# soedinglab/BaMMmotif2

Hardware: AMD Instinct MI355X
Metric: EM seq-positions/sec (and iterations/sec), 1Mx200bp k=2 W=20 (higher is better)
Workload: dtype f32

## Files before the change

### bammmotif2_amd/build.py

```python
from __future__ import annotations

import contextlib
import fcntl
import json
import os
import re
import shutil
import subprocess

HERE = os.path.dirname(os.path.abspath(__file__))
CSRC = os.path.join(HERE, "csrc")
LIB = os.path.join(HERE, "libbamm_em.so")
SOURCES = ["model.hip", "kernels.hip", "grouped.hip", "grouped_long.hip", "grouped_xl.hip", "grouped_mix.hip", "grouped_mix1.hip", "mask.hip", "seed.hip", "long_seq.hip", "prep.hip", "negs.hip", "occ.hip", "sites.hip", "fdr.hip", "ctx.cpp", "seqs.cpp", "plan.cpp", "em_pass.cpp", "em.cpp",
           "score.cpp", "occurrences.cpp", "sites.cpp", "fdr_stats.cpp", "comm.cpp", "pack.cpp"]
HEADERS = [os.path.join(CSRC, "common.h"), os.path.join(CSRC, "device_utils.h"), os.path.join(CSRC, "grouped_kernel.h"), os.path.join(CSRC, "mixed_kernel.h"), os.path.join(CSRC, "update_kernel.h"), os.path.join(CSRC, "phase_clock.h"),
           os.path.join(HERE, "..", "include", "bamm_em.h")]
FLAGS = ["--offload-arch=gfx950", "-O3", "-std=c++17", "-fPIC", "-ffp-contract=off", "-fno-slp-vectorize",
         "-Wall", "-Wno-unused-result", "-Rpass-analysis=kernel-resource-usage"]
_IEEE = ["-fhip-fp32-correctly-rounded-divide-sqrt", "-fno-gpu-flush-denormals-to-zero"]
TU_FLAGS = {"occ.hip": _IEEE, "fdr.hip": _IEEE, "grouped_long.hip": ["-falign-functions=16384"], "grouped_xl.hip": ["-falign-functions=16384"], "kernels.hip": ["-falign-functions=16384"]}
OBJDIR = os.path.join(HERE, "build")
RESOURCES = os.path.join(OBJDIR, "resources.json")


def _stem(src: str) -> str:
    stem, ext = os.path.splitext(src)
    return stem + "_host" if ext == ".cpp" and stem + ".hip" in SOURCES else stem


def _obj(src: str) -> str:
    return os.path.join(OBJDIR, _stem(src) + ".o")


def _remarks(src: str) -> str:
    return os.path.join(OBJDIR, _stem(src) + ".remarks")


def _diagnostics(text: str) -> str:
    keep, skip = [], 0
    for line in text.splitlines():
        if "[-Rpass-analysis=kernel-resource-usage]" in line:
            skip = 2 if "Function Name" in line else 0
            continue
        if skip:
            skip -= 1
            continue
        keep.append(line)
    return "\n".join(keep).strip()
# ... 166 lines not shown
```

### bammmotif2_amd/csrc/common.h

```cpp
#pragma once
#include <hip/hip_runtime.h>

#include <cstdint>
#include <cstdio>
#include <cstring>
#include <map>
#include <memory>
#include <string>
#include <vector>

#include "../../include/bamm_em.h"

namespace bamm {

void set_error(const char* fmt, ...);

#define BAMM_HIP(expr)                                                                        \
    do {                                                                                      \
        hipError_t e_ = (expr);                                                               \
        if (e_ != hipSuccess) {                                                               \
            ::bamm::set_error("%s failed: %s (%s:%d)", #expr, hipGetErrorString(e_), __FILE__, \
                              __LINE__);                                                      \
            return BAMM_ERR_HIP;                                                              \
        }                                                                                     \
// ... 122 lines not shown
    const float* v_old;
    float* s;
    float* q;
    float* q_out;
    float* status;
    float* trace;
    uint32_t trace_cap;
    uint32_t* iteration;
    int32_t optimize_q;
    double n_seqs_override;
    uint32_t* stop;
    float epsilon;
    float llh_prev;
    int32_t llh_prev_from_status;
    const float* llh_in;
    float* llh_out;
    uint32_t opt_iteration;
    unsigned long long* status_mirror;
    double*   partial;
    uint32_t* ticket;
};
constexpr uint32_t kUpdateMaxBlocks = 1024;

inline size_t update_lds_bytes(uint32_t K, uint32_t W) {
    auto even = [](size_t x) { return (x + 1) & ~size_t(1); };
    return (even(v_size(K, W)) + even((size_t)(K + 1) * W) + even(bg_size(K))) * sizeof(float) + (16 + 4) * sizeof(double);
}
inline bool update_fits_lds(uint32_t K, uint32_t W) { return ipow4(K + 1) * W <= 2048u && update_lds_bytes(K, W) <= 60u * 1024u; }

struct GrpKernelArgs {
    EmKernelArgs e;
    GrpGeom g;
    const uint4* xrec;
    unsigned long long* fix_log;
    uint32_t fix_log_cap;
    uint32_t fused;
    uint32_t upd_off;
    float*   s_block;
    UpdateArgs upd;
    PeerArgs peer;
};

bool grp_geometry(uint32_t K, uint32_t W, uint32_t G, int M, uint32_t waves, bool accum, uint32_t logC, uint32_t layout,
                  GrpGeom* out);
bool grp_plan(uint32_t K, uint32_t W, int M, uint32_t waves, bool many_exceptions, bool enough_work, uint32_t forced_G,
              int forced_layout, uint32_t* G, uint32_t* logC, uint32_t* layout);
bool grp_supported_class(int M, uint32_t K);
int launch_em_grp_long(int mclass, bool accum, bool write_r, const GrpKernelArgs& a, uint32_t blocks, uint32_t threads,
                       hipStream_t st);
int launch_em_grp_xl(int mclass, bool accum, bool write_r, const GrpKernelArgs& a, uint32_t blocks, uint32_t threads,
                     hipStream_t st);
uint32_t grp_max_threads(int M);
bool mix_geometry(uint32_t K, uint32_t W, int M, uint32_t waves, bool accum, GrpGeom* out);
int launch_em_mix(int mclass, bool accum, bool write_r, const GrpKernelArgs& a, uint32_t blocks, uint32_t threads, hipStream_t st);
int launch_em_mix1(int mclass, bool accum, bool write_r, const GrpKernelArgs& a, uint32_t blocks, uint32_t threads, hipStream_t st);
int launch_em_grp(int mclass, bool accum, bool write_r, const GrpKernelArgs& a, uint32_t blocks, uint32_t threads,
                  hipStream_t st);

struct SeedKernelArgs {
    SeqView  sv;
    uint32_t K, W, Y;
    uint32_t max_len, vsize;
    uint32_t table_bytes, count_bytes, wave_bytes;
    const float* score;
    float    q;
    const double* u;
    int*     counts;
    uint32_t* z_out;
    unsigned char* wave_scratch;
};
size_t seed_global_scratch_bytes(const SeedKernelArgs& a, uint32_t num_cus);
int launch_seed_pwm(SeedKernelArgs a, uint32_t num_cus, hipStream_t st);

struct ScoreKernelArgs {
    SeqView  sv;
    uint32_t K, W, Y;
    const float* s;
    float*   mops;
    const uint64_t* mops_off;
    float*   zoops;
    uint32_t* z;
};


struct OccCand {
    unsigned long long window;
    float    score;
    float    higher, lower;
    uint32_t fp;
};
// ... 134 lines not shown
```

### bammmotif2_amd/csrc/em.cpp

```cpp

#include <atomic>
#include <cmath>

#include "handles.h"

using namespace bamm;

int bamm::dense_r_on_device(bamm_em* em, uint64_t begin, uint64_t end, DevTemps& tmp, DenseR* out) {
    bamm_seqs* s = em->seqs;
    hipStream_t st = em->ctx->stream;
    const uint64_t base = s->h_pos_off[begin], total = s->h_pos_off[end] - base;
    if (em->mask_done) {
        *out = DenseR{em->d_mask_r, 0, false};
        return BAMM_OK;
    }
    if (em->sliced) {
        uint8_t* saved_mask = em->d_mask;
        em->d_mask = nullptr;
        const uint32_t used = em->events_used, pass_no = em->pass_no;
        int rc2 = run_accumulate(em, false, true, true);
        em->events_used = used; em->pass_no = pass_no;
        em->d_mask = saved_mask;
        if (rc2) return rc2;
        *out = DenseR{em->d_state, 0, !em->e_fused};
// ... 3 lines not shown
    int rc = tmp.scratch(&d_r, total);
    if (rc) return rc;
    if (hipMemsetAsync(d_r, 0, total * sizeof(float), st) != hipSuccess) { set_error("hipMemsetAsync failed"); return BAMM_ERR_HIP; }
    for (size_t b = 0; b < em->ebuckets.size() && !rc; b++) {
        const EmBucket& bk = em->ebuckets[b];
        EmKernelArgs a{};
        a.sv = make_view(s, em->exc, bk.d_idx, bk.count, nullptr);
        a.K = em->prm.K; a.W = em->prm.W; a.Y = em->Y;
        a.s = em->s_last; a.q = em->q_last;
        a.acc = nullptr;
        a.r_out = d_r; a.r_base = base; a.seq_begin = (uint32_t)begin; a.seq_end = (uint32_t)end;
        a.fix_scale = 1.0f;
        if (bk.mclass == kLongClass) { rc = launch_long_em(a, false, true, false, bk.blocks, st); continue; }
        rc = launch_fused(em, bk, false, true, a, bucket_threads(em->ctx, bk), st);
    }
    *out = DenseR{d_r, base, false};
    return rc;
}

extern "C" {

int bamm_em_destroy(bamm_em* em) {
    if (!em) return BAMM_OK;
    (void)hipSetDevice(em->ctx->device);
    (void)hipStreamSynchronize(em->ctx->stream);
    for (void* p : {(void*)em->d_vbg, (void*)em->d_A, (void*)em->d_v, (void*)em->d_n, (void*)em->d_s, (void*)em->d_qbuf[0],
                    (void*)em->d_status, (void*)em->d_trace, (void*)em->d_iteration, (void*)em->d_mask, (void*)em->d_acc_ring,
                    (void*)em->d_v_alt, (void*)em->d_llh[0], (void*)em->d_s_block, (void*)em->d_nnz, (void*)em->d_upd_partial, (void*)em->d_upd_ticket,
                    (void*)em->d_state, (void*)em->d_list_r, (void*)em->d_list_p, (void*)em->d_list_n, (void*)em->d_s_alt, (void*)em->d_fix_log,
                    (void*)em->d_qbuf[1], (void*)em->d_qbuf[2],
                    (void*)em->d_mask_r, (void*)em->d_mask_bits, (void*)em->d_mask_hist, (void*)em->d_mask_sel, (void*)em->d_mask_qseq,
                    (void*)em->d_mask_partial_n, (void*)em->d_mask_partial_stat})
        scratch_free(em->ctx, p);
    for (uint32_t* p : em->owned_idx) (void)hipFree(p);
    if (em->h_status) (void)hipHostFree(em->h_status);
    (void)hipFree(em->d_stop);
    (void)hipFree(em->d_peer_words);
    (void)hipFree(em->d_comm_words);
    for (hipEvent_t e : em->opt_events) if (e) (void)hipEventDestroy(e);
    for (auto& ev : em->events) { (void)hipEventDestroy(ev.first); (void)hipEventDestroy(ev.second); }
    bamm_seqs_destroy(em->seqs);
    delete em;
    return BAMM_OK;
}

int bamm_em_create(bamm_ctx* c, bamm_seqs* seqs, const bamm_em_params* prm, const float* vbg, const float* A,
                   const float* v_init, const uint8_t* seq_mask, bamm_em** out) {
    if (!c || !seqs || !prm || !vbg || !A || !v_init || !out) { set_error("bamm_em_create: null argument"); return BAMM_ERR_ARG; }
    *out = nullptr;
    if (seqs->ctx != c) { set_error("sequence set belongs to another context"); return BAMM_ERR_ARG; }
    if (prm->K > BAMM_MAX_ORDER) { set_error("order %u > %d (kmer_ spans 11 bases)", prm->K, BAMM_MAX_ORDER); return BAMM_ERR_ARG; }
    if (prm->W == 0) { set_error("motif width 0"); return BAMM_ERR_ARG; }
    if (seqs->n && seqs->min_len < prm->W) {
        set_error("a sequence of length %u is shorter than the motif (W=%u); the reference drops those before EM (mainBaMM.cpp:75-83)",
                  seqs->min_len, prm->W);
        return BAMM_ERR_ARG;
    }
    const uint32_t Y = (uint32_t)ipow4(prm->K + 1);
    BAMM_HIP(hipSetDevice(c->device));
    bamm_em* em = new bamm_em();
    em->ctx = c;
    em->seqs = seqs;
    { std::lock_guard<std::mutex> lock(seqs->mu); seqs->refs++; }
    em->prm = *prm;
    if (em->prm.max_iterations == 0) em->prm.max_iterations = 1000;
    em->Y = Y;
// ... 562 lines not shown
```

### bammmotif2_amd/csrc/em_pass.cpp

```cpp

#include <cmath>

#include "handles.h"

namespace bamm {

static int event_pair(bamm_em* em) {
    if (em->events_used == em->events.size()) {
        hipEvent_t a, b;
        BAMM_HIP(hipEventCreate(&a));
        BAMM_HIP(hipEventCreate(&b));
        em->events.emplace_back(a, b);
        em->event_passes.push_back(1u);
    }
    return BAMM_OK;
}
int record_event(bamm_em* em, bool start) {
    if (em->timing_every == BAMM_TIMING_WHOLE_CALL) {
        if (!start) return BAMM_OK;
        em->pass_no++;
        if (!em->region_open) {
            if (int rc = event_pair(em)) return rc;
            BAMM_HIP(hipEventRecord(em->events[em->events_used].first, em->ctx->stream));
            em->region_open = true;
// ... 9 lines not shown
    if (!em->timing_now) return BAMM_OK;
    if (start) {
        if (int rc = event_pair(em)) return rc;
        BAMM_HIP(hipEventRecord(em->events[em->events_used].first, em->ctx->stream));
    } else {
        BAMM_HIP(hipEventRecord(em->events[em->events_used].second, em->ctx->stream));
        em->event_passes[em->events_used] = 1u;
        em->events_used++;
    }
    return BAMM_OK;
}
int close_timed_region(bamm_em* em) {
    if (!em->region_open) return BAMM_OK;
    em->region_open = false;
    BAMM_HIP(hipEventRecord(em->events[em->events_used].second, em->ctx->stream));
    em->event_passes[em->events_used] = em->region_passes;
    em->events_used++;
    return BAMM_OK;
}

int launch_fused(bamm_em* em, const EmBucket& eb, bool accum, bool write_r, EmKernelArgs& a, uint32_t threads,
                 hipStream_t st, const UpdateArgs* fuse) {
    if (!eb.grouped) {
        a.logC = eb.logc;
        a.sparse_cap = accum ? eb.sparse_cap : 0u;
        a.sparse_wave_bytes = accum ? eb.sparse_bytes : 0u;
        return launch_em_seq(eb.mclass, accum, write_r, a, eb.blocks, threads, st);
    }
    GrpKernelArgs ga{};
    a.logC = eb.logc;
    a.sparse_cap = 0; a.sparse_wave_bytes = 0;
    ga.e = a;
    ga.xrec = eb.d_xrec;
    if (!grp_geometry(em->prm.K, em->prm.W, eb.G, kMClasses[eb.mclass], threads / 64u, accum, accum ? eb.logc : 0u, eb.layout, &ga.g)) {
        set_error("grouped kernel geometry does not fit (K=%u W=%u)", em->prm.K, em->prm.W);
        return BAMM_ERR_UNSUPPORTED;
    }
    if ((em->prm.K == 3u || (eb.layout & 8u)) && accum) {
        const size_t waves = (size_t)eb.blocks * (threads / 64u);
        const size_t cap = ((eb.count + waves - 1) / waves) * std::min<size_t>(64, (size_t)ga.g.Bv * ga.g.T);
        const size_t need = waves * cap;
        if (need > em->fix_log_words) {
            if (em->d_fix_log) { scratch_free(em->ctx, em->d_fix_log); em->d_fix_log = nullptr; em->fix_log_words = 0; }
            if (int rc = scratch_alloc(em->ctx, &em->d_fix_log, need)) return rc;
            em->fix_log_words = need;
        }
        ga.fix_log = em->d_fix_log;
        ga.fix_log_cap = (uint32_t)cap;
    }
    if (fuse) {
        ga.fused = 1u; ga.upd = *fuse; ga.upd_off = em->fuse_upd_off; ga.s_block = em->d_s_block;
    }
    if (em->peer_on && accum && !write_r) {
        em->pass_summed_in_kernel = true;
        comm_peer_args(em->comm, &ga.peer);
        ga.peer.words = (uint32_t)em->cells + 3u;
        ga.peer.ticket = em->d_peer_words; ga.peer.err = em->d_peer_words + 1;
        ga.peer.timeout_ticks = (unsigned long long)em->ctx->peer_timeout_ms * 100000ull;
        ga.peer.seq = comm_peer_next_seq(em->comm);
        ga.peer.slot = (uint32_t)(ga.peer.seq % 3ull);
    }
    return launch_em_grp(eb.mclass, accum, write_r, ga, eb.blocks, threads, st);
}

static EmBook capture_book(const bamm_em* em) {
    return EmBook{em->d_s, em->d_s_alt, em->d_q, em->d_v, em->d_v_alt, em->s_last, em->q_last, em->d_acc, em->acc_cur, em->llh_cur,
// ... 281 lines not shown
```

### bammmotif2_amd/csrc/handles.h

```cpp
#pragma once

#include <algorithm>
#include <mutex>
#include <thread>
#include <unordered_map>

#include "common.h"
#include "prep.h"

#ifndef BAMM_FUSE_MAX_M
#define BAMM_FUSE_MAX_M 16
#endif

namespace bamm {

template <class T>
struct NoInitAlloc : std::allocator<T> {
    template <class U> struct rebind { using other = NoInitAlloc<U>; };
    template <class U, class... A> void construct(U* p, A&&... a) {
        if constexpr (sizeof...(A) == 0) ::new ((void*)p) U; else ::new ((void*)p) U(std::forward<A>(a)...);
    }
};
template <class T> using RawVec = std::vector<T, NoInitAlloc<T>>;

struct Bucket {
    int mclass = 0;
    uint32_t count = 0;
    uint32_t* d_idx = nullptr;
    std::vector<uint32_t> h_idx;
    double work = 0;
};

struct ExcK {
    uint64_t* d_off = nullptr;
    uint2* d_exc = nullptr;
    uint64_t count = 0;
    RawVec<uint64_t> h_off;
    RawVec<uint2> h_ex;
    struct XRec {
        uint4* d_xrec = nullptr;
        RawVec<uint8_t> h_B;
        RawVec<uint32_t> h_lo;
    };
    std::map<uint32_t, XRec> xrec;
};

struct EmBucket {
    int mclass = 0;
    uint32_t count = 0;
    const uint32_t* d_idx = nullptr;
    bool grouped = false;
    uint32_t G = 0;
    uint32_t layout = 0;
    const uint4* d_xrec = nullptr;
    uint32_t blocks = 0, logc = 0, sparse_cap = 0, sparse_bytes = 0;
    double work = 0;
};

struct EmBook {
    float *d_s, *d_s_alt, *d_q, *d_v, *d_v_alt; const float *s_last, *q_last;
    long long* d_acc; uint32_t acc_cur, llh_cur, host_iteration, events_used, pass_no;
    bool estep_done, acc_dirty, mask_done, ring_prev_dirty;
};

}

struct bamm_ctx {
    int device = 0;
    hipStream_t stream = nullptr;
    bool own_stream = false;
    uint32_t blocks = 0, threads = 0;
    bool use_grouped = true, use_sparse = true, use_e_fused = true, use_e_list = true, use_fused_update = true, use_adaptive_lists = true, use_update_blocks = true;
    uint32_t list_threshold_pct = 45;
    uint32_t group_size = 0;
    int group_layout = -1;
    bool use_peer_allreduce = false;
    uint32_t peer_timeout_ms = 2000;
    int num_cus = 0;
    std::string name;
    std::mutex scratch_mu;
    std::unordered_map<void*, size_t> scratch_live;
    std::vector<std::pair<void*, size_t>> scratch_idle;
    size_t scratch_idle_bytes = 0, scratch_cap_bytes = 0;
    uint32_t sites_chunk_positions = 0;
    bool scratch_poison = false;
    uint64_t scratch_hits = 0, scratch_misses = 0;
    std::mutex stage_mu;
// ... 45 lines not shown
    float *d_q = nullptr, *d_status = nullptr, *d_trace = nullptr;
    float *d_s_alt = nullptr;
    float *d_qbuf[3] = {nullptr, nullptr, nullptr};
    const float *s_last = nullptr, *q_last = nullptr;
    uint32_t* d_iteration = nullptr;
    uint8_t* d_mask = nullptr;
    long long* d_acc = nullptr;
    long long* d_acc_ring = nullptr;
    size_t acc_stride = 0;
    uint32_t acc_cur = 0;
    bool fusable = false;
    uint32_t fuse_upd_off = 0;
    float* d_s_block = nullptr;
    float* d_v_alt = nullptr;
    float* d_llh[2] = {nullptr, nullptr};
    double* d_upd_partial = nullptr;
    uint32_t* d_upd_ticket = nullptr;
    uint32_t llh_cur = 0;
    bool ring_prev_dirty = false;
    bool acc_external = false;
    bool acc_dirty = false;
    uint32_t fix_shift = 40;
    float* h_status = nullptr;
    unsigned long long* h_tagged = nullptr;
    unsigned long long* d_status_mirror = nullptr;
    uint32_t* d_stop = nullptr;
    const uint32_t* stop_arg = nullptr;
    hipEvent_t opt_events[2] = {nullptr, nullptr};
    uint32_t opt_iteration = 0;
    float opt_llh_prev = 0.0f;
    uint32_t total_blocks = 0;
    std::vector<bamm::EmBucket> ebuckets;
    std::vector<uint32_t*> owned_idx;
    uint32_t threads = 0;
    bool sliced = false;
    std::vector<std::pair<uint32_t, uint32_t>> e_slices, m_slices;
    uint32_t m_slice_logc = 0;
    bool e_fused = false;
    uint32_t m_slice_cap = 0;
    float* d_state = nullptr;
    float* d_list_r = nullptr;
    uint16_t* d_list_p = nullptr;
    uint32_t* d_list_n = nullptr;
    unsigned long long* d_nnz = nullptr;
    uint32_t nnz_prev_slot = 0;
    unsigned long long nnz_limit = 0;
    bool adaptive_lists = true;
    unsigned long long* d_fix_log = nullptr;
    size_t fix_log_words = 0;
    bamm::ExcK* exc = nullptr;
    bool estep_done = false;
    float llh_prev = 0.0f;
    uint32_t host_iteration = 0;
    bamm_allreduce_fn allreduce = nullptr;
    void* allreduce_user = nullptr;
    bamm_comm* comm = nullptr;
    bool comm_verified = false;
    bool peer_on = false;
    bool pass_summed_in_kernel = false;
    uint32_t* d_peer_words = nullptr;
    long long* d_comm_words = nullptr;
    std::string peer_note;
    std::vector<std::pair<hipEvent_t, hipEvent_t>> events;
    uint32_t events_used = 0;
    uint32_t timing_every = 8, pass_no = 0;
    bool timing_now = false;
// ... 121 lines not shown
```

### bammmotif2_amd/csrc/mixed_kernel.h

```cpp
#pragma once
#include "grouped_kernel.h"

namespace bamm {
namespace {

constexpr uint32_t kMixBj = 6u, kMixNe = 3u, kMixBv = kMixBj + kMixNe;

template <int OFF>
__device__ __forceinline__ void lds_add_u64_exec_big(uint32_t byte_addr, unsigned long long v, unsigned long long mask) {
    static_assert(OFF >= 0 && OFF < 65536, "ds offset field");
    lds_add_u64_exec<OFF>(byte_addr, v, mask);
}

template <int M, int A, int NQ, bool ACCUM, bool WRITE_R, int THREADS>
__global__ void __launch_bounds__(THREADS) k_em_mix(GrpKernelArgs ga) {
    static_assert(M >= 4 && 2 * (M - 1) + 12 <= 32, "a wide group within one lane's run, rows out of one stream window");
    static_assert(A == 1 || A == 2, "wide groups");
    constexpr uint32_t WAVES = THREADS / 64, V = WAVES * kMixBv;
    constexpr uint32_t R5N = 1024u, R5V0 = R5N + 1u, R5T = R5V0 + V;
    constexpr uint32_t R6N = 4096u, R6V0 = R6N + 1u, R6T = R6V0 + V;
    constexpr uint32_t Y = 64u, Ys = 65u;
    if (ga.e.stop != nullptr && *ga.e.stop != 0u) return;
    extern __shared__ __align__(16) unsigned char lds_raw[];
    BAMM_PHASE(0);
    const EmKernelArgs& a = ga.e;
    const GrpGeom& g = ga.g;
    const uint32_t W = a.W, T = g.T, B = g.mixB;
    const uint32_t pad = 4u * NQ - B;
    const uint32_t rs5 = g.rowstride;
    float* sg5 = reinterpret_cast<float*>(lds_raw + g.off_sg);
    float* sg6 = reinterpret_cast<float*>(lds_raw + g.off_sg6);
    const float* s1_stage = reinterpret_cast<const float*>(lds_raw + g.off_s1);
    double* stat_lds = reinterpret_cast<double*>(lds_raw + g.off_stat);
    unsigned long long* cnt5 = reinterpret_cast<unsigned long long*>(lds_raw + g.off_ng);
    unsigned long long* cnt6 = reinterpret_cast<unsigned long long*>(lds_raw + g.off_ng6);
    unsigned long long* n1 = reinterpret_cast<unsigned long long*>(lds_raw + g.off_n1);
    unsigned long long* n1p = reinterpret_cast<unsigned long long*>(lds_raw + g.off_wave);
    const uint32_t n1c = ACCUM ? g.wave_bytes / (Y * 8u) : 0u;

    const int lane = threadIdx.x & 63;
    const uint32_t wave = __builtin_amdgcn_readfirstlane(threadIdx.x >> 6);
    const uint32_t total_waves = gridDim.x * WAVES;
    uint32_t t = blockIdx.x * WAVES + wave;
    RawSeqG<M> nxt{};
    if (t < a.sv.count) nxt = fetch_seq_g<M>(a.sv, ga.xrec, t, lane);

    [[maybe_unused]] float q_fused = 0.0f;
    {
        float* s1w = reinterpret_cast<float*>(lds_raw + g.off_s1);
        const float* s1 = s1_stage;
        bool staged = false;
        if constexpr (ACCUM) {
            if (ga.fused) {
                const UpdateOut uo = model_update_lds<false>(ga.upd, lds_raw + ga.upd_off, s1w, blockIdx.x == 0);
                if (uo.fired) {
                    if (blockIdx.x == 0) { __syncthreads(); publish_odds(ga.upd, s1w, nullptr, true); }
                    return;
                }
                q_fused = uo.q;
                staged = true;
            }
        }
        BAMM_PHASE(1);
        if (!staged)
            for (uint32_t i = threadIdx.x; i < W * Ys; i += THREADS) s1w[i] = a.s[i];
        for (uint32_t i = threadIdx.x; i < (R5T - R5N) * rs5; i += THREADS) sg5[R5N * rs5 + i] = 1.0f;
        for (uint32_t i = threadIdx.x; i < (R6T - R6N) * A; i += THREADS) sg6[R6N * A + i] = 1.0f;
        __syncthreads();
        if constexpr (ACCUM)
            if (staged) publish_odds(ga.upd, s1w, ga.s_block + (size_t)blockIdx.x * (W * Ys), blockIdx.x == 0);
        for (uint32_t row = threadIdx.x; row < R5N; row += THREADS) {
            float* out = sg5 + row * rs5;
            for (uint32_t slot = 0; slot < pad; slot++) out[slot] = 1.0f;
            for (uint32_t slot = pad + B; slot < rs5; slot++) out[slot] = 1.0f;
            for (uint32_t tt = 0; tt < B; tt++) {
                float f = 1.0f;
#pragma unroll
                for (int c = 0; c < 3; c++) f *= s1[(3u * tt + c) * Ys + ((row >> (2 * (2 - c))) & 63u)];
                out[pad + tt] = f;
            }
        }
        for (uint32_t row = threadIdx.x; row < R6N; row += THREADS) {
#pragma unroll
            for (int w = 0; w < A; w++) {
                float f = 1.0f;
#pragma unroll
                for (int c = 0; c < 4; c++) f *= s1[(3u * B + 4u * w + c) * Ys + ((row >> (2 * (3 - c))) & 63u)];
                sg6[row * A + w] = f;
            }
        }
        __syncthreads();
        if (ACCUM) {
            for (uint32_t i = threadIdx.x; i < B * R5T; i += THREADS) cnt5[i] = 0ull;
            for (uint32_t i = threadIdx.x; i < A * R6T; i += THREADS) cnt6[i] = 0ull;
            for (uint32_t i = threadIdx.x; i < n1c * Y; i += THREADS) n1p[i] = 0ull;
            __syncthreads();
        }
    }

    BAMM_PHASE(2);
    if constexpr (ACCUM) {
        const __attribute__((address_space(4))) GrpKernelArgs* kq =
            (const __attribute__((address_space(4))) GrpKernelArgs*)__builtin_amdgcn_kernarg_segment_ptr();
        asm volatile("" : "+s"(kq));
        if (kq->peer.world > 1u && *kq->peer.err != 0u) return;
    }
    const float q = (ACCUM && ga.fused) ? q_fused : *a.q;
    const float one_minus_q = 1.0f - q;
    const uint32_t lane_b = (uint32_t)lane / T, lane_t = (uint32_t)lane - lane_b * T;
    const bool lane_wide = lane_t >= B;
    const uint32_t lane_G = lane_wide ? 4u : 3u;
    const uint32_t lane_col0 = lane_wide ? 3u * B + 4u * (lane_t - B) : 3u * lane_t;
    const uint32_t vbase5 = R5V0 + wave * kMixBv, vbase6 = R6V0 + wave * kMixBv;
    const uint32_t sg5_base = lds_offset(sg5), sg6_base = lds_offset(sg6);

    uint32_t resident_fill = 0u;
#pragma unroll
    for (int c = 0; c < 4; c++)
        if (lane_col0 + (uint32_t)c < n1c) resident_fill |= Y << (7 * c);
    double llh_acc = 0.0, sumr_acc = 0.0;
    uint32_t seq_cnt = 0, last_LW1 = 0;
    float pos_i = 0.0f;
    float pos_m[M];
    constexpr bool kCacheSpec = M <= 7 || THREADS < 1024;
    [[maybe_unused]] int spec[kCacheSpec ? M : 1];
    [[maybe_unused]] uint32_t spec_LW1 = 0, spec_xw = 0xffffffffu;
#pragma unroll
    for (int m = 0; m < M; m++) pos_m[m] = 0.0f;
#pragma unroll
    for (int m = 0; m < (kCacheSpec ? M : 1); m++) spec[m] = -1;
    [[maybe_unused]] GrpLogEntry* my_log = nullptr;
    [[maybe_unused]] uint32_t nlog = 0;
    if constexpr (ACCUM)
        my_log = reinterpret_cast<GrpLogEntry*>(ga.fix_log) + (size_t)(blockIdx.x * WAVES + wave) * ga.fix_log_cap;

    for (; t < a.sv.count; t += total_waves) {
        const RawSeqG<M> cur = nxt;
        const __attribute__((address_space(4))) GrpKernelArgs* kp =
            (const __attribute__((address_space(4))) GrpKernelArgs*)__builtin_amdgcn_kernarg_segment_ptr();
        asm volatile("" : "+s"(kp));
        if (t + total_waves < a.sv.count) {
            SeqView sv2;
            sv2.words = kp->e.sv.words; sv2.word_off = kp->e.sv.word_off; sv2.len = kp->e.sv.len; sv2.pos_off = nullptr;
            sv2.exc_off = nullptr; sv2.exc = nullptr; sv2.mask = kp->e.sv.mask; sv2.idx = kp->e.sv.idx; sv2.count = a.sv.count;
            nxt = fetch_seq_g<M>(sv2, kp->xrec, t + total_waves, lane);
        }
        const uint32_t seq = cur.seq;
        if (WRITE_R && (seq < a.seq_begin || seq >= a.seq_end)) continue;
        if (!cur.ok) continue;
        __builtin_amdgcn_s_setprio(0);
        const uint32_t L = __builtin_amdgcn_readfirstlane(cur.L);
        const uint32_t LW1 = L - W + 1u;
        const uint32_t p0 = (uint32_t)lane * M;

        uint32_t X, sE;
        {
            constexpr int NSEL = RawSeqG<M>::NSEL;
            const uint32_t wi0 = p0 >> 4;
            const uint32_t pE = LW1 - 1u, lpE = pE / (uint32_t)M;
            const uint32_t pe = p0 + (uint32_t)(M - 1);
            const uint32_t sel = (pe >> 4) - wi0;
            uint32_t lo = cur.w[1], hi = cur.w[0];
#pragma unroll
            for (int c = 1; c < NSEL; c++) {
                lo = (sel == (uint32_t)c) ? cur.w[c + 1] : lo;
                hi = (sel == (uint32_t)c) ? cur.w[c] : hi;
            }
            X = __builtin_amdgcn_alignbit(hi, lo, 30u - 2u * (pe & 15u));
            sE = (uint32_t)__builtin_amdgcn_readlane((int)X, (int)lpE) >> (2u * ((uint32_t)(M - 1) - (pE - lpE * (uint32_t)M)));
        }

        const uint32_t xw = __builtin_amdgcn_readfirstlane(cur.xr.x);
        const uint32_t Bx = (xw >> 12) & 0xfu;
        const uint32_t xlo = xw & 0xfffu;
        const uint32_t nE = min(kMixNe, L - LW1);
        uint32_t yfix = Y | (Y << 7) | (Y << 14) | (Y << 21);
        const bool fixJ = lane_b < Bx;
        const bool fixE = lane_b >= kMixBj && lane_b < kMixBj + nE;
        const bool fix = fixJ || fixE;
        float fs[4] = {1.0f, 1.0f, 1.0f, 1.0f};
        const float* const sfix_now = (ACCUM && kp->fused) ? kp->s_block + (size_t)blockIdx.x * (W * Ys) : kp->e.s;
        if (fix) {
            const uint32_t pv = fixJ ? xlo + lane_b : LW1 + (lane_b - kMixBj);
            const uint32_t xfields = xrec_fields<7>(cur.xr.y, cur.xr.z, cur.xr.w, lane_b + 4u - lane_G);
#pragma unroll
            for (int c = 0; c < 4; c++) {
                uint32_t yc = Y;
                const uint32_t colc = min(lane_col0 + (uint32_t)c, W - 1u);
                if ((uint32_t)c < lane_G) {
                    const uint32_t pos = pv - (lane_G - 1u) + (uint32_t)c;
                    if (fixJ) {
                        yc = (xfields >> (7u * (uint32_t)c)) & 0x7fu;
                    } else {
                        yc = (sE >> (2u * ((LW1 - 1u - pos) & 15u))) & (Y - 1u);
                    }
                    if (pos >= LW1) yc = Y;
                }
                yfix = (yfix & ~(0x7fu << (7 * c))) | (yc << (7 * c));
                fs[c] = sfix_now[__umul24(colc, Ys) + yc];
            }
        }
        auto slot_offsets = [&](int (&o)[M]) {
#pragma unroll
            for (int m = 0; m < M; m++) {
                const uint32_t k2 = p0 + m - xlo, k3 = p0 + m - LW1;
                o[m] = (p0 + m < LW1) ? -1 : 0;
                if (k2 < Bx) o[m] = (int)(1u + wave * kMixBv + k2);
                if (k3 < nE) o[m] = (int)(1u + wave * kMixBv + kMixBj + k3);
            }
        };
        uint32_t row5[M], row6[M];
        if constexpr (kCacheSpec) {
            if (LW1 != spec_LW1 || xw != spec_xw) {
                spec_LW1 = LW1; spec_xw = xw;
                slot_offsets(spec);
            }
#pragma unroll
            for (int m = 0; m < M; m++) {
                const bool stream = spec[m] < 0;
                row5[m] = stream ? ((X >> (2 * (M - 1 - m))) & 1023u) : R5N + (uint32_t)spec[m];
                row6[m] = stream ? ((X >> (2 * (M - 1 - m))) & 4095u) : R6N + (uint32_t)spec[m];
            }
        } else {
            int o[M];
            slot_offsets(o);
#pragma unroll
            for (int m = 0; m < M; m++) {
                const bool stream = o[m] < 0;
                row5[m] = stream ? ((X >> (2 * (M - 1 - m))) & 1023u) : R5N + (uint32_t)o[m];
                row6[m] = stream ? ((X >> (2 * (M - 1 - m))) & 4095u) : R6N + (uint32_t)o[m];
            }
        }
// ... 279 lines not shown
```

### bammmotif2_amd/csrc/plan.cpp

```cpp

#include <atomic>
#include <cmath>

#include "handles.h"

namespace bamm {

namespace {

constexpr size_t kLds = 160 * 1024;

int prime_bucket(bamm_ctx* c, const bamm_em_params& prm, uint32_t Y, bool sliced, const EmBucket& eb) {
    if (hipSetDevice(c->device) != hipSuccess) { set_error("hipSetDevice failed"); return BAMM_ERR_HIP; }
    EmKernelArgs a{};
    a.K = prm.K; a.W = prm.W; a.Y = Y;
    if (eb.mclass == kLongClass) return launch_long_em(a, true, false, false, kPrimeOnly, c->stream);
    const uint32_t threads = bucket_threads(c, eb);
    if (sliced || !eb.grouped) {
        a.logC = 0;
        return launch_em_seq(eb.mclass, false, false, a, kPrimeOnly, threads, c->stream);
    }
    GrpKernelArgs ga{};
    ga.e = a;
    if (!grp_geometry(prm.K, prm.W, eb.G, kMClasses[eb.mclass], threads / 64u, true, eb.logc, eb.layout, &ga.g)) return BAMM_OK;
    return launch_em_grp(eb.mclass, true, false, ga, kPrimeOnly, threads, c->stream);
}

}

uint32_t default_threads(const bamm_ctx* c, int mclass) {
    uint32_t t = c->threads ? c->threads : max_threads_for_mclass(mclass);
    return std::min(t, max_threads_for_mclass(mclass));
}

uint32_t bucket_threads(const bamm_ctx* c, const EmBucket& b) {
    if (b.mclass == kLongClass) return 256u;
    const uint32_t t = default_threads(c, b.mclass);
    return b.grouped ? std::min(t, grp_max_threads(kMClasses[b.mclass])) : t;
}

uint32_t default_blocks(const bamm_ctx* c, uint32_t threads) {
    if (c->blocks) return c->blocks;
    const uint32_t cus = c->num_cus > 0 ? (uint32_t)c->num_cus : 256u;
    return cus * std::max(1u, 2048u / threads);
}

bool plan_slices(bamm_em* em) {
    const bamm_em_params* prm = &em->prm;
    const bamm_ctx* c = em->ctx;
    const uint32_t Y = em->Y;
    bool sliced = em_lds_bytes(prm->W, Y, true, 0, 0) > kLds;
    uint32_t e_cols = 0, m_cols = 0;
    bool global_tables = false;
    if (sliced) {
        while (e_cols < prm->W && e_slice_lds_bytes(e_cols + 1, Y) <= kLds) e_cols++;
        while (m_cols < prm->W && m_slice_lds_bytes(m_cols + 1, Y, 0) <= kLds) m_cols++;
        if (e_cols == 0 || m_cols == 0) { global_tables = true; sliced = false; }
// ... 62 lines not shown
            }
            with_exc_a.fetch_add(cnt, std::memory_order_relaxed);
        });
        const size_t with_exc = with_exc_a.load();
        if (want_grouped && grp_supported_class(Mcls, prm->K) &&
            grp_plan(prm->K, prm->W, Mcls, std::min(threads, grp_max_threads(Mcls)) / 64u, 2 * with_exc > b.count, plan_n * (uint64_t)Mcls >= 40000ull * 7ull, c->group_size, c->group_layout, &gG, &glogc, &glayout) &&
            grp_geometry(prm->K, prm->W, gG, Mcls, std::min(threads, grp_max_threads(Mcls)) / 64u, true, glogc, glayout, &gg)) {
            { EmBucket pb; pb.mclass = b.mclass; pb.grouped = true; pb.logc = glogc; pb.G = gG; pb.layout = glayout; prime(pb); }
            if ((rc = xrec_for_group(seqs, prm->K, gG, em->exc, &xr))) return rc;
            auto capable = [&](uint32_t n) {
                const uint32_t B = xr->h_B[n];
                return B == 0u || (B <= gg.Bj && (gg.np != 0u || xr->h_lo[n] + B + gg.G <= seqs->h_len[n] - prm->W + 1u));
            };
            std::atomic<bool> all_capable{true};
            host_ranges(b.count, [&](uint64_t i0, uint64_t i1) {
                for (uint64_t i = i0; i < i1 && all_capable.load(std::memory_order_relaxed); i++)
                    if (!capable(b.d_idx ? b.h_idx[i] : (uint32_t)i)) all_capable.store(false, std::memory_order_relaxed);
            });
            const bool all = all_capable.load();
            if (!all)
                for (uint32_t i = 0; i < b.count; i++) {
                    const uint32_t n = b.d_idx ? b.h_idx[i] : i;
                    (capable(n) ? yes : no).push_back(n);
                }
            EmBucket eb;
            eb.mclass = b.mclass; eb.grouped = true; eb.logc = glogc; eb.G = gG; eb.layout = glayout; eb.d_xrec = xr->d_xrec;
            if (all) { eb.count = b.count; eb.d_idx = b.d_idx; }
            else {
                uint32_t* d = nullptr;
                if ((rc = dev_upload(c, &d, yes.data(), yes.size()))) return rc;
                em->owned_idx.push_back(d);
                eb.count = (uint32_t)yes.size(); eb.d_idx = d;
            }
            eb.work = (double)eb.count * Mcls * 0.6;
            if (eb.count) em->ebuckets.push_back(eb);
            if (all) continue;
        }
        EmBucket eb;
        eb.mclass = b.mclass;
        if (!no.empty()) {
            uint32_t* d = nullptr;
            if ((rc = dev_upload(c, &d, no.data(), no.size()))) return rc;
            em->owned_idx.push_back(d);
            eb.count = (uint32_t)no.size(); eb.d_idx = d;
        } else { eb.count = b.count; eb.d_idx = b.d_idx; }
        eb.work = (double)eb.count * Mcls;
        em->ebuckets.push_back(eb);
        prime(eb);
    }
    if (!em->owned_idx.empty() && hipStreamSynchronize(st) != hipSuccess) { set_error("stream sync failed"); return BAMM_ERR_HIP; }
    double total_work = 0;
    for (auto& b : em->ebuckets) total_work += b.work;
    em->total_blocks = 0;
    for (auto& b : em->ebuckets) {
        if (b.mclass == kLongClass) {
            b.blocks = std::min(b.count, (uint32_t)std::max(1, c->num_cus) * 8u);
            em->total_blocks += b.blocks;
            continue;
        }
        const uint32_t threads = bucket_threads(c, b);
        const uint32_t blocks_per_cu = sliced ? 1u : std::max(1u, 1024u / threads);
        if (!b.grouped) {
            const int Mcls = kMClasses[b.mclass];
            size_t scratch = sliced ? 0 : sparse_wave_bytes(Mcls) * (threads / 64u);
            uint32_t cap = sliced ? 0u : sparse_cap_for(Mcls);
            if (!c->use_sparse) { cap = 0; scratch = 0; }
// ... 59 lines not shown
```

Measured before the change: 484.4 billion.

## Precompute per-lane mixed-kernel records once at plan time

Adds a setup kernel that computes, for every sequence and lane, the packed sequence word X and the fix-up column codes used by the mixed-row EM kernel, and stores them as a uint2 array. The EM kernel then loads one 8-byte record per lane instead of fetching raw sequence words and redoing the select/alignbit/readlane and exception decoding every iteration. This trades extra device memory (64 records per sequence) and a one-time preprocessing pass for less per-iteration ALU and sequence-load work. Records are built from sequence data, which stays fixed across EM iterations.

```diff
diff --git a/bammmotif2_amd/build.py b/bammmotif2_amd/build.py
--- a/bammmotif2_amd/build.py
+++ b/bammmotif2_amd/build.py
@@ -11,9 +11,9 @@
 HERE = os.path.dirname(os.path.abspath(__file__))
 CSRC = os.path.join(HERE, "csrc")
 LIB = os.path.join(HERE, "libbamm_em.so")
-SOURCES = ["model.hip", "kernels.hip", "grouped.hip", "grouped_long.hip", "grouped_xl.hip", "grouped_mix.hip", "grouped_mix1.hip", "mask.hip", "seed.hip", "long_seq.hip", "prep.hip", "negs.hip", "occ.hip", "sites.hip", "fdr.hip", "ctx.cpp", "seqs.cpp", "plan.cpp", "em_pass.cpp", "em.cpp",
+SOURCES = ["model.hip", "kernels.hip", "grouped.hip", "grouped_long.hip", "grouped_xl.hip", "grouped_mix.hip", "grouped_mix1.hip", "lane_records.hip", "mask.hip", "seed.hip", "long_seq.hip", "prep.hip", "negs.hip", "occ.hip", "sites.hip", "fdr.hip", "ctx.cpp", "seqs.cpp", "plan.cpp", "em_pass.cpp", "em.cpp",
            "score.cpp", "occurrences.cpp", "sites.cpp", "fdr_stats.cpp", "comm.cpp", "pack.cpp"]
-HEADERS = [os.path.join(CSRC, "common.h"), os.path.join(CSRC, "device_utils.h"), os.path.join(CSRC, "grouped_kernel.h"), os.path.join(CSRC, "mixed_kernel.h"), os.path.join(CSRC, "update_kernel.h"), os.path.join(CSRC, "phase_clock.h"),
+HEADERS = [os.path.join(CSRC, "common.h"), os.path.join(CSRC, "device_utils.h"), os.path.join(CSRC, "grouped_kernel.h"), os.path.join(CSRC, "mixed_kernel.h"), os.path.join(CSRC, "lane_records.h"), os.path.join(CSRC, "update_kernel.h"), os.path.join(CSRC, "phase_clock.h"),
            os.path.join(HERE, "..", "include", "bamm_em.h")]
 FLAGS = ["--offload-arch=gfx950", "-O3", "-std=c++17", "-fPIC", "-ffp-contract=off", "-fno-slp-vectorize",
          "-Wall", "-Wno-unused-result", "-Rpass-analysis=kernel-resource-usage"]
diff --git a/bammmotif2_amd/csrc/common.h b/bammmotif2_amd/csrc/common.h
--- a/bammmotif2_amd/csrc/common.h
+++ b/bammmotif2_amd/csrc/common.h
@@ -178,6 +178,7 @@
     EmKernelArgs e;
     GrpGeom g;
     const uint4* xrec;
+    const uint2* lane_rec;
     unsigned long long* fix_log;
     uint32_t fix_log_cap;
     uint32_t fused;
@@ -202,6 +203,8 @@
 int launch_em_mix1(int mclass, bool accum, bool write_r, const GrpKernelArgs& a, uint32_t blocks, uint32_t threads, hipStream_t st);
 int launch_em_grp(int mclass, bool accum, bool write_r, const GrpKernelArgs& a, uint32_t blocks, uint32_t threads,
                   hipStream_t st);
+int launch_mix_records(int mclass, const SeqView& sv, const uint4* xrec, uint32_t W, uint32_t T, uint32_t B, uint2* out,
+                       uint32_t num_cus, hipStream_t st);
 
 struct SeedKernelArgs {
     SeqView  sv;
diff --git a/bammmotif2_amd/csrc/em.cpp b/bammmotif2_amd/csrc/em.cpp
--- a/bammmotif2_amd/csrc/em.cpp
+++ b/bammmotif2_amd/csrc/em.cpp
@@ -59,6 +59,7 @@
                     (void*)em->d_mask_r, (void*)em->d_mask_bits, (void*)em->d_mask_hist, (void*)em->d_mask_sel, (void*)em->d_mask_qseq,
                     (void*)em->d_mask_partial_n, (void*)em->d_mask_partial_stat})
         scratch_free(em->ctx, p);
+    for (uint2* p : em->owned_lane_rec) scratch_free(em->ctx, p);
     for (uint32_t* p : em->owned_idx) (void)hipFree(p);
     if (em->h_status) (void)hipHostFree(em->h_status);
     (void)hipFree(em->d_stop);
diff --git a/bammmotif2_amd/csrc/em_pass.cpp b/bammmotif2_amd/csrc/em_pass.cpp
--- a/bammmotif2_amd/csrc/em_pass.cpp
+++ b/bammmotif2_amd/csrc/em_pass.cpp
@@ -65,6 +65,7 @@
     a.sparse_cap = 0; a.sparse_wave_bytes = 0;
     ga.e = a;
     ga.xrec = eb.d_xrec;
+    ga.lane_rec = eb.d_lane_rec;
     if (!grp_geometry(em->prm.K, em->prm.W, eb.G, kMClasses[eb.mclass], threads / 64u, accum, accum ? eb.logc : 0u, eb.layout, &ga.g)) {
         set_error("grouped kernel geometry does not fit (K=%u W=%u)", em->prm.K, em->prm.W);
         return BAMM_ERR_UNSUPPORTED;
diff --git a/bammmotif2_amd/csrc/handles.h b/bammmotif2_amd/csrc/handles.h
--- a/bammmotif2_amd/csrc/handles.h
+++ b/bammmotif2_amd/csrc/handles.h
@@ -53,6 +53,7 @@
     uint32_t G = 0;
     uint32_t layout = 0;
     const uint4* d_xrec = nullptr;
+    const uint2* d_lane_rec = nullptr;
     uint32_t blocks = 0, logc = 0, sparse_cap = 0, sparse_bytes = 0;
     double work = 0;
 };
@@ -164,6 +165,7 @@
     uint32_t total_blocks = 0;
     std::vector<bamm::EmBucket> ebuckets;
     std::vector<uint32_t*> owned_idx;
+    std::vector<uint2*> owned_lane_rec;
     uint32_t threads = 0;
     bool sliced = false;
     std::vector<std::pair<uint32_t, uint32_t>> e_slices, m_slices;
diff --git a/bammmotif2_amd/csrc/lane_records.h b/bammmotif2_amd/csrc/lane_records.h
--- /dev/null
+++ b/bammmotif2_amd/csrc/lane_records.h
@@ -0,0 +1,82 @@
+#pragma once
+#include "grouped_kernel.h"
+
+namespace bamm {
+namespace {
+
+constexpr uint32_t kMixBj = 6u, kMixNe = 3u, kMixBv = kMixBj + kMixNe;
+constexpr uint32_t kMixFixBit = 1u << 31;
+
+template <int M>
+__device__ __forceinline__ uint2 mix_lane_record(const RawSeqG<M>& cur, int lane, uint32_t W, uint32_t T, uint32_t B) {
+    constexpr uint32_t Y = 64u;
+    const uint32_t L = __builtin_amdgcn_readfirstlane(cur.L);
+    const uint32_t LW1 = L - W + 1u;
+    const uint32_t p0 = (uint32_t)lane * M;
+
+    uint32_t X, sE;
+    {
+        constexpr int NSEL = RawSeqG<M>::NSEL;
+        const uint32_t wi0 = p0 >> 4;
+        const uint32_t pE = LW1 - 1u, lpE = pE / (uint32_t)M;
+        const uint32_t pe = p0 + (uint32_t)(M - 1);
+        const uint32_t sel = (pe >> 4) - wi0;
+        uint32_t lo = cur.w[1], hi = cur.w[0];
+#pragma unroll
+        for (int c = 1; c < NSEL; c++) {
+            lo = (sel == (uint32_t)c) ? cur.w[c + 1] : lo;
+            hi = (sel == (uint32_t)c) ? cur.w[c] : hi;
+        }
+        X = __builtin_amdgcn_alignbit(hi, lo, 30u - 2u * (pe & 15u));
+        sE = (uint32_t)__builtin_amdgcn_readlane((int)X, (int)lpE) >> (2u * ((uint32_t)(M - 1) - (pE - lpE * (uint32_t)M)));
+    }
+
+    const uint32_t lane_b = (uint32_t)lane / T, lane_t = (uint32_t)lane - lane_b * T;
+    const uint32_t lane_G = lane_t >= B ? 4u : 3u;
+    const uint32_t xw = __builtin_amdgcn_readfirstlane(cur.xr.x);
+    const uint32_t Bx = (xw >> 12) & 0xfu;
+    const uint32_t xlo = xw & 0xfffu;
+    const uint32_t nE = min(kMixNe, L - LW1);
+    uint32_t yfix = Y | (Y << 7) | (Y << 14) | (Y << 21);
+    const bool fixJ = lane_b < Bx;
+    const bool fixE = lane_b >= kMixBj && lane_b < kMixBj + nE;
+    if (fixJ || fixE) {
+        const uint32_t pv = fixJ ? xlo + lane_b : LW1 + (lane_b - kMixBj);
+        const uint32_t xfields = xrec_fields<7>(cur.xr.y, cur.xr.z, cur.xr.w, lane_b + 4u - lane_G);
+#pragma unroll
+        for (int c = 0; c < 4; c++) {
+            uint32_t yc = Y;
+            if ((uint32_t)c < lane_G) {
+                const uint32_t pos = pv - (lane_G - 1u) + (uint32_t)c;
+                if (fixJ) {
+                    yc = (xfields >> (7u * (uint32_t)c)) & 0x7fu;
+                } else {
+                    yc = (sE >> (2u * ((LW1 - 1u - pos) & 15u))) & (Y - 1u);
+                }
+                if (pos >= LW1) yc = Y;
+            }
+            yfix = (yfix & ~(0x7fu << (7 * c))) | (yc << (7 * c));
+        }
+        yfix |= kMixFixBit;
+    }
+    return make_uint2(X, yfix);
+}
+
+struct MixSeq {
+    uint32_t seq, L, xw;
+    uint2 rec;
+    bool ok;
+};
+
+__device__ __forceinline__ MixSeq fetch_mix_seq(const SeqView& sv, const uint4* xrec, const uint2* lane_rec, uint32_t t, int lane) {
+    MixSeq r;
+    r.rec = lane_rec[(size_t)t * 64u + (uint32_t)lane];
+    r.seq = pick_sequence(sv, t);
+    r.ok = !(sv.mask && !sv.mask[r.seq]);
+    r.L = sv.len[r.seq];
+    r.xw = reinterpret_cast<const uint32_t*>(xrec + r.seq)[0];
+    return r;
+}
+
+}
+}
diff --git a/bammmotif2_amd/csrc/lane_records.hip b/bammmotif2_amd/csrc/lane_records.hip
--- /dev/null
+++ b/bammmotif2_amd/csrc/lane_records.hip
@@ -0,0 +1,47 @@
+#include <algorithm>
+
+#include "lane_records.h"
+
+namespace bamm {
+namespace {
+
+constexpr uint32_t kRecThreads = 256u, kRecWaves = kRecThreads / 64u;
+
+template <int M>
+__global__ void __launch_bounds__(kRecThreads) k_mix_records(SeqView sv, const uint4* xrec, uint32_t W, uint32_t T, uint32_t B, uint2* out) {
+    const int lane = threadIdx.x & 63;
+    const uint32_t total_waves = gridDim.x * kRecWaves;
+    for (uint32_t t = blockIdx.x * kRecWaves + (threadIdx.x >> 6); t < sv.count; t += total_waves) {
+        const RawSeqG<M> cur = fetch_seq_g<M>(sv, xrec, t, lane);
+        out[(size_t)t * 64u + (uint32_t)lane] = mix_lane_record<M>(cur, lane, W, T, B);
+    }
+}
+
+template <int M>
+int launch_records(const SeqView& sv, const uint4* xrec, uint32_t W, uint32_t T, uint32_t B, uint2* out, uint32_t blocks, hipStream_t st) {
+    return launch_kernel(&k_mix_records<M>, blocks, kRecThreads, 0, st, sv, xrec, W, T, B, out);
+}
+
+}
+
+int launch_mix_records(int mclass, const SeqView& sv, const uint4* xrec, uint32_t W, uint32_t T, uint32_t B, uint2* out,
+                       uint32_t num_cus, hipStream_t st) {
+    if (sv.count == 0u && num_cus != kPrimeOnly) return BAMM_OK;
+    const uint32_t blocks = num_cus == kPrimeOnly ? kPrimeOnly
+                                                  : std::min((sv.count + kRecWaves - 1u) / kRecWaves, std::max(1u, num_cus) * 8u);
+    int rc = BAMM_ERR_UNSUPPORTED;
+    switch (mclass) {
+        case 3: rc = launch_records<4>(sv, xrec, W, T, B, out, blocks, st); break;
+        case 4: rc = launch_records<5>(sv, xrec, W, T, B, out, blocks, st); break;
+        case 5: rc = launch_records<6>(sv, xrec, W, T, B, out, blocks, st); break;
+        case 6: rc = launch_records<7>(sv, xrec, W, T, B, out, blocks, st); break;
+        case 7: rc = launch_records<8>(sv, xrec, W, T, B, out, blocks, st); break;
+        case 8: rc = launch_records<10>(sv, xrec, W, T, B, out, blocks, st); break;
+        default: set_error("no mixed-row kernel for M class %d", mclass);
+    }
+    if (rc) return rc;
+    if (blocks != kPrimeOnly) BAMM_HIP(hipGetLastError());
+    return BAMM_OK;
+}
+
+}
diff --git a/bammmotif2_amd/csrc/mixed_kernel.h b/bammmotif2_amd/csrc/mixed_kernel.h
--- a/bammmotif2_amd/csrc/mixed_kernel.h
+++ b/bammmotif2_amd/csrc/mixed_kernel.h
@@ -1,10 +1,8 @@
 #pragma once
-#include "grouped_kernel.h"
+#include "lane_records.h"
 
 namespace bamm {
 namespace {
-
-constexpr uint32_t kMixBj = 6u, kMixNe = 3u, kMixBv = kMixBj + kMixNe;
 
 template <int OFF>
 __device__ __forceinline__ void lds_add_u64_exec_big(uint32_t byte_addr, unsigned long long v, unsigned long long mask) {
@@ -42,8 +40,8 @@
     const uint32_t wave = __builtin_amdgcn_readfirstlane(threadIdx.x >> 6);
     const uint32_t total_waves = gridDim.x * WAVES;
     uint32_t t = blockIdx.x * WAVES + wave;
-    RawSeqG<M> nxt{};
-    if (t < a.sv.count) nxt = fetch_seq_g<M>(a.sv, ga.xrec, t, lane);
+    MixSeq nxt{};
+    if (t < a.sv.count) nxt = fetch_mix_seq(a.sv, ga.xrec, ga.lane_rec, t, lane);
 
     [[maybe_unused]] float q_fused = 0.0f;
     {
@@ -109,7 +107,6 @@
     const float one_minus_q = 1.0f - q;
     const uint32_t lane_b = (uint32_t)lane / T, lane_t = (uint32_t)lane - lane_b * T;
     const bool lane_wide = lane_t >= B;
-    const uint32_t lane_G = lane_wide ? 4u : 3u;
     const uint32_t lane_col0 = lane_wide ? 3u * B + 4u * (lane_t - B) : 3u * lane_t;
     const uint32_t vbase5 = R5V0 + wave * kMixBv, vbase6 = R6V0 + wave * kMixBv;
     const uint32_t sg5_base = lds_offset(sg5), sg6_base = lds_offset(sg6);
@@ -135,15 +132,15 @@
         my_log = reinterpret_cast<GrpLogEntry*>(ga.fix_log) + (size_t)(blockIdx.x * WAVES + wave) * ga.fix_log_cap;
 
     for (; t < a.sv.count; t += total_waves) {
-        const RawSeqG<M> cur = nxt;
+        const MixSeq cur = nxt;
         const __attribute__((address_space(4))) GrpKernelArgs* kp =
             (const __attribute__((address_space(4))) GrpKernelArgs*)__builtin_amdgcn_kernarg_segment_ptr();
         asm volatile("" : "+s"(kp));
         if (t + total_waves < a.sv.count) {
             SeqView sv2;
-            sv2.words = kp->e.sv.words; sv2.word_off = kp->e.sv.word_off; sv2.len = kp->e.sv.len; sv2.pos_off = nullptr;
+            sv2.words = nullptr; sv2.word_off = nullptr; sv2.len = kp->e.sv.len; sv2.pos_off = nullptr;
             sv2.exc_off = nullptr; sv2.exc = nullptr; sv2.mask = kp->e.sv.mask; sv2.idx = kp->e.sv.idx; sv2.count = a.sv.count;
-            nxt = fetch_seq_g<M>(sv2, kp->xrec, t + total_waves, lane);
+            nxt = fetch_mix_seq(sv2, kp->xrec, kp->lane_rec, t + total_waves, lane);
         }
         const uint32_t seq = cur.seq;
         if (WRITE_R && (seq < a.seq_begin || seq >= a.seq_end)) continue;
@@ -153,51 +150,19 @@
         const uint32_t LW1 = L - W + 1u;
         const uint32_t p0 = (uint32_t)lane * M;
 
-        uint32_t X, sE;
-        {
-            constexpr int NSEL = RawSeqG<M>::NSEL;
-            const uint32_t wi0 = p0 >> 4;
-            const uint32_t pE = LW1 - 1u, lpE = pE / (uint32_t)M;
-            const uint32_t pe = p0 + (uint32_t)(M - 1);
-            const uint32_t sel = (pe >> 4) - wi0;
-            uint32_t lo = cur.w[1], hi = cur.w[0];
-#pragma unroll
-            for (int c = 1; c < NSEL; c++) {
-                lo = (sel == (uint32_t)c) ? cur.w[c + 1] : lo;
-                hi = (sel == (uint32_t)c) ? cur.w[c] : hi;
-            }
-            X = __builtin_amdgcn_alignbit(hi, lo, 30u - 2u * (pe & 15u));
-            sE = (uint32_t)__builtin_amdgcn_readlane((int)X, (int)lpE) >> (2u * ((uint32_t)(M - 1) - (pE - lpE * (uint32_t)M)));
-        }
-
-        const uint32_t xw = __builtin_amdgcn_readfirstlane(cur.xr.x);
+        const uint32_t X = cur.rec.x, yfix = cur.rec.y;
+        const bool fix = (int)yfix < 0;
+        const uint32_t xw = __builtin_amdgcn_readfirstlane(cur.xw);
         const uint32_t Bx = (xw >> 12) & 0xfu;
         const uint32_t xlo = xw & 0xfffu;
         const uint32_t nE = min(kMixNe, L - LW1);
-        uint32_t yfix = Y | (Y << 7) | (Y << 14) | (Y << 21);
-        const bool fixJ = lane_b < Bx;
-        const bool fixE = lane_b >= kMixBj && lane_b < kMixBj + nE;
-        const bool fix = fixJ || fixE;
         float fs[4] = {1.0f, 1.0f, 1.0f, 1.0f};
         const float* const sfix_now = (ACCUM && kp->fused) ? kp->s_block + (size_t)blockIdx.x * (W * Ys) : kp->e.s;
         if (fix) {
-            const uint32_t pv = fixJ ? xlo + lane_b : LW1 + (lane_b - kMixBj);
-            const uint32_t xfields = xrec_fields<7>(cur.xr.y, cur.xr.z, cur.xr.w, lane_b + 4u - lane_G);
 #pragma unroll
             for (int c = 0; c < 4; c++) {
-                uint32_t yc = Y;
                 const uint32_t colc = min(lane_col0 + (uint32_t)c, W - 1u);
-                if ((uint32_t)c < lane_G) {
-                    const uint32_t pos = pv - (lane_G - 1u) + (uint32_t)c;
-                    if (fixJ) {
-                        yc = (xfields >> (7u * (uint32_t)c)) & 0x7fu;
-                    } else {
-                        yc = (sE >> (2u * ((LW1 - 1u - pos) & 15u))) & (Y - 1u);
-                    }
-                    if (pos >= LW1) yc = Y;
-                }
-                yfix = (yfix & ~(0x7fu << (7 * c))) | (yc << (7 * c));
-                fs[c] = sfix_now[__umul24(colc, Ys) + yc];
+                fs[c] = sfix_now[__umul24(colc, Ys) + ((yfix >> (7 * c)) & 0x7fu)];
             }
         }
         auto slot_offsets = [&](int (&o)[M]) {
diff --git a/bammmotif2_amd/csrc/plan.cpp b/bammmotif2_amd/csrc/plan.cpp
--- a/bammmotif2_amd/csrc/plan.cpp
+++ b/bammmotif2_amd/csrc/plan.cpp
@@ -23,6 +23,8 @@
     GrpKernelArgs ga{};
     ga.e = a;
     if (!grp_geometry(prm.K, prm.W, eb.G, kMClasses[eb.mclass], threads / 64u, true, eb.logc, eb.layout, &ga.g)) return BAMM_OK;
+    if (eb.layout & 8u)
+        if (int rc = launch_mix_records(eb.mclass, SeqView{}, nullptr, prm.W, ga.g.T, ga.g.mixB, nullptr, kPrimeOnly, c->stream)) return rc;
     return launch_em_grp(eb.mclass, true, false, ga, kPrimeOnly, threads, c->stream);
 }
 
@@ -151,6 +153,14 @@
                 em->owned_idx.push_back(d);
                 eb.count = (uint32_t)yes.size(); eb.d_idx = d;
             }
+            if ((glayout & 8u) && eb.count) {
+                uint2* rec = nullptr;
+                if ((rc = scratch_alloc(c, &rec, (size_t)eb.count * 64u))) return rc;
+                em->owned_lane_rec.push_back(rec);
+                if ((rc = launch_mix_records(eb.mclass, make_view(seqs, em->exc, eb.d_idx, eb.count, nullptr), xr->d_xrec, prm->W,
+                                             gg.T, gg.mixB, rec, (uint32_t)std::max(1, c->num_cus), st))) return rc;
+                eb.d_lane_rec = rec;
+            }
             eb.work = (double)eb.count * Mcls * 0.6;
             if (eb.count) em->ebuckets.push_back(eb);
             if (all) continue;
```

After: 500.5 billion (median of 6 runs). 3.3% higher.
